# chen-zichen/distributed_learning_simulator

Measured on AMD Instinct MI355X. Metric: client-update GB/s aggregated per FL round + Shapley subset-evals/sec, higher is better.
Workload: dtype fp32; 1 GPU; FedAvg aggregation of 100 synthetic ResNet-18 (11.2M-param fp32) client updates (per GPU), bit-exact reference order; parallelism=clients sharded over 1 GPU(s) + RCCL all-reduce, clients_per_gpu=100, clients_total=100, params=11173962, padded_row=11174016

## Files before the change

### distributed_learning_simulator_amd/_native.py

```python
import ctypes
import os
import threading

import torch

_HERE = os.path.dirname(os.path.abspath(__file__))
LIB_PATH = os.environ.get("DLS_HIP_LIB", os.path.join(_HERE, "libdls_hip.so"))

FEDAVG_EXACT = 0
FEDAVG_FMA = 1
SIGN_NAN_MARK = 1 << 24
QTILE_GROUPS = 10
SUBSET_UNION_MAX = 64


def sign_words(P):
    return ((P + 255) // 256) * 8


def sign_row_pitch(P):
    return (sign_words(P) + 15) // 16 * 16


class QTile(ctypes.Structure):
# ... 31 lines not shown
    "dls_sign_sgd_direction": ([_p, _p, _i64, _f32, _f32, _i32, _i32, _p, _p, _p], _i32),
    "dls_sign_sgd_apply": ([_p, _p, _i64, _f32, _f32, _p], _i32),
    "dls_dequant_fedavg": ([_p, _i32, _p, _p, _i64, _p, _i64, _p, _i64, _i64, _p, _p, _i32, _f32,
                            _p, _p],
                           _i32),
    "dls_dequant_fedavg_mode": ([_p, _i32, _p, _p, _i64, _p, _i64, _p, _i64, _i64, _p, _p, _i32,
                                 _f32, _i32, _p, _p], _i32),
    "dls_segment_minmax_f32": ([_p, _p, _i32, _p, _p, _i64, _p], _i32),
    "dls_qparams_minmax": ([_p, _p, _i32, _i32, _i32, _i32, _p, _p, _p], _i32),
    "dls_quantize_affine": ([_p, _p, _i32, _p, _p, _i32, _i32, _p, _p, _i32, _u64, _i64, _p],
                            _i32),
    "dls_bn_fold_f32": ([_p, _p, _p, _p, _f32, _i32, _p, _p, _p], _i32),
    "dls_bn_act_nhwc_f32": ([_p, _i64, _i32, _p, _p, _p, _i32, _p, _p], _i32),
    "dls_bn_fold_exact_f32": ([_p, _p, _p, _p, _f32, _i32, _p, _p], _i32),
    "dls_bn_act_exact_nhwc_f32": ([_p, _i64, _i32, _p, _p, _i32, _p, _p], _i32),
    "dls_bn_act_exact_nchw_f32": ([_p, _i64, _i32, _i64, _p, _p, _i32, _p, _p], _i32),
    "dls_conv_pack_input_f32": ([_p, _i64, _i32, _i32, _i32, _i32, _p, _p], _i32),
    "dls_conv_pack_weights_f32": ([_p, _i32, _i32, _i32, _i32, _i32, _p, _p], _i32),
    "dls_conv_pack_im2col_f32": ([_p, _i64, _i32, _i32, _i32, _i32, _i32, _i32, _i32, _i32, _p, _p],
                                 _i32),
    "dls_conv_pack_weights_im2col_f32": ([_p, _i32, _i32, _i32, _i32, _i32, _p, _p], _i32),
    "dls_conv_bn_act_split": ([_p, _i64, _i32, _i32, _i32, _p, _i32, _i32, _i32, _i32, _i32, _p, _p,
                               _i32, _p, _p], _i32),
    "dls_conv_stem_bn_act_f32": ([_p, _i64, _i32, _i32, _i32, _p, _i32, _i32, _i32, _i32, _i32, _p,
                                  _i32, _p, _p], _i32),
    "dls_pool_linear_split": ([_p, _i64, _i32, _i32, _p, _p, _i32, _p, _p], _i32),
    "dls_conv_kernel_choice": ([_i64, _i32, _i32, _i32, _i32, _i32, _i32, _i32, _i32], _i32),
    "dls_conv_stem_kernel_choice": ([_i64, _i32, _i32, _i32, _i32, _i32, _i32, _i32, _i32], _i32),
    "dls_lenet5_eval_f32": ([_p, _i64, _i32, _p, _p, _i64, _p, _i32, _p, _p, _p], _i32),
    "dls_lenet5_eval_loss_f32": ([_p, _i64, _i32, _p, _p, _i64, _p, _i32, _p, _p, _p, _i64, _p],
                                 _i32),
    "dls_softmax_ce_f32": ([_p, _i32, _i64, _i32, _p, _p, _i64, _p], _i32),
    "dls_sum_rows_f64": ([_p, _i64, _i32, _i64, _p, _p], _i32),
}

_lib = None
_lock = threading.Lock()


def lib():
    global _lib
    if _lib is None:
        with _lock:
            if _lib is None:
                if not os.path.exists(LIB_PATH):
                    raise RuntimeError(
# ... 242 lines not shown
        return
    if (consts.dtype != torch.float32 or consts.numel() != 4 * cout or not consts.is_contiguous()
            or consts.device != device):
        raise RuntimeError(f"{fn}: consts must be a contiguous fp32 tensor of 4 * Cout = {4 * cout} "
                           f"elements on {device}")


def _overlaps(a, b):
    a0 = a.data_ptr()
    b0 = b.data_ptr()
    return a0 < b0 + b.numel() * b.element_size() and b0 < a0 + a.numel() * a.element_size()


def split_channels(c):
    return (int(c) + 31) // 32 * 32


CONV_KERNELS = {
    0: "none", 1: "generic<1,4>", 2: "generic<2,2>", 3: "pipe<1,4,10,1,2>", 4: "pipe<1,4,12,1,2>",
    5: "pipe<2,2,5,1,2>", 6: "pipe<2,4,5>", 7: "pipe<2,4,6>", 8: "halo<2,2,9,false>",
    9: "halo<2,2,9,true>", 10: "halo<1,4,11,false>", 11: "halo<1,4,11,true>", 12: "phase<2,4,5>",
}
STEM_KERNELS = {0: "none", 1: "window", 2: "3x3", 3: "generic"}


def conv_kernel_choice(B, H, W, C, Cout, ksize, stride, pad):
    kh, kw = ksize
    return int(lib().dls_conv_kernel_choice(B, H, W, C, Cout, kh, kw, stride, pad))


def conv_stem_kernel_choice(B, C, H, W, Cout, ksize, stride, pad):
    kh, kw = ksize
    return int(lib().dls_conv_stem_kernel_choice(B, C, H, W, Cout, kh, kw, stride, pad))


def conv_pack_input(x, stream=None):
    if x.dtype != torch.float32 or x.dim() != 4 or not x.is_contiguous():
        raise RuntimeError("conv_pack_input: x must be a contiguous NCHW fp32 tensor")
    B, C, H, W = x.shape
    cp = split_channels(C)
    out = torch.empty((B, H, W, 2 * cp), dtype=torch.int16, device=x.device)
    _check(lib().dls_conv_pack_input_f32(_ptr(x), B, C, H, W, cp, _ptr(out), _stream(stream, x)),
           "dls_conv_pack_input_f32")
    return out


def conv_pack_weights(w, stream=None):
    w = w.detach()
    if w.dtype != torch.float32 or w.dim() != 4 or not w.is_contiguous():
        raise RuntimeError("conv_pack_weights: w must be a contiguous fp32 [Cout, Cin, KH, KW]")
    co, ci, kh, kw = w.shape
    cp = split_channels(ci)
    out = torch.empty((co, 2 * kh * kw * cp), dtype=torch.int16, device=w.device)
    _check(lib().dls_conv_pack_weights_f32(_ptr(w), co, ci, kh, kw, cp, _ptr(out),
                                           _stream(stream, w)), "dls_conv_pack_weights_f32")
    return out
# ... 36 lines not shown
        raise RuntimeError(f"conv_bn_act: weights {tuple(w.shape)} do not match input channels {c2 // 2}")
    _check_same_device("conv_bn_act", x, w=w)
    _check_consts("conv_bn_act", consts, cout, x.device)
    oshape = (B, ho, wo, 2 * cout)
    if residual is not None:
        if (tuple(residual.shape) != oshape or residual.dtype != torch.int16
                or not residual.is_contiguous()):
            raise RuntimeError("conv_bn_act: residual must be a contiguous split NHWC int16 tensor "
                               "of the output's shape")
        _check_same_device("conv_bn_act", x, residual=residual)
    if out is None:
        out = torch.empty(oshape, dtype=torch.int16, device=x.device)
    else:
        if tuple(out.shape) != oshape or out.dtype != torch.int16 or not out.is_contiguous():
            raise RuntimeError(f"conv_bn_act: out must be a contiguous int16 tensor of shape {oshape}")
        _check_same_device("conv_bn_act", x, out=out)
        for name, t in (("x", x), ("residual", residual)):
            if t is not None and _overlaps(out, t):
                raise RuntimeError(f"conv_bn_act: out must not alias {name}")
    _check(lib().dls_conv_bn_act_split(_ptr(x), B, H, W, c2 // 2, _ptr(w), cout, kh, kw, stride,
                                       pad, _ptr(consts), _ptr(residual), int(bool(relu)),
                                       _ptr(out), _stream(stream, x)), "dls_conv_bn_act_split")
    return out


def conv_stem_bn_act(x, w, ksize, stride, pad, consts=None, relu=True, stream=None):
    if x.dtype != torch.float32 or x.dim() != 4 or not x.is_contiguous():
        raise RuntimeError("conv_stem_bn_act: x must be a contiguous NCHW fp32 tensor")
    B, C, H, W = x.shape
    kh, kw = ksize
    cout = w.shape[0]
    if w.dtype != torch.int16 or w.shape[1] != 2 * 32 or not w.is_contiguous():
        raise RuntimeError("conv_stem_bn_act: w must be conv_pack_weights_im2col output with Kp = 32")
    _check_same_device("conv_stem_bn_act", x, w=w)
    _check_consts("conv_stem_bn_act", consts, cout, x.device)
    ho, wo = (H + 2 * pad - kh) // stride + 1, (W + 2 * pad - kw) // stride + 1
    out = torch.empty((B, ho, wo, 2 * cout), dtype=torch.int16, device=x.device)
    _check(lib().dls_conv_stem_bn_act_f32(_ptr(x), B, C, H, W, _ptr(w), cout, kh, kw, stride, pad,
                                          _ptr(consts), int(bool(relu)), _ptr(out),
                                          _stream(stream, x)), "dls_conv_stem_bn_act_f32")
    return out


def pool_linear(x, weight, bias=None, stream=None):
    B, H, W, c2 = x.shape
    if x.dtype != torch.int16 or not x.is_contiguous():
# ... 131 lines not shown
```

### distributed_learning_simulator_amd/csrc/conv.hip

```cpp
#include "dls_common.h"

#include <mutex>

#ifndef DLS_CONV_GENERIC_ONLY
#define DLS_CONV_GENERIC_ONLY 0
#endif
#ifndef DLS_CONV_PHASE
#define DLS_CONV_PHASE 1
#endif
#ifndef DLS_STEM_WINDOW
#define DLS_STEM_WINDOW 1
#endif
#ifndef DLS_CONV_MF16
#define DLS_CONV_MF16 1
#endif
#ifndef DLS_STEM_TILES
#define DLS_STEM_TILES 2
#endif
#ifndef DLS_CONV_SERPENTINE
#define DLS_CONV_SERPENTINE 1
#endif
#ifndef DLS_PIPE_NARROW
#define DLS_PIPE_NARROW 1
#endif
// ... 30 lines not shown
typedef __attribute__((ext_vector_type(2))) float f32x2;

__device__ __forceinline__ void split2x2(float a, float b, uint32_t &hi2, uint32_t &lo2) {
    hi2 = __builtin_bit_cast(uint32_t, __builtin_convertvector(f32x2{a, b}, bf16x2));
    float ra = a - __uint_as_float(hi2 << 16);
    float rb = b - __uint_as_float(hi2 & 0xffff0000u);
    ra = (__float_as_uint(ra) & 0x7f800000u) == 0x7f800000u ? 0.f : ra;
    rb = (__float_as_uint(rb) & 0x7f800000u) == 0x7f800000u ? 0.f : rb;
    lo2 = __builtin_bit_cast(uint32_t, __builtin_convertvector(f32x2{ra, rb}, bf16x2));
}

struct ConvArgs {
    const uint16_t *x;
    const uint16_t *w;
    const float *consts;
    const uint16_t *res;
    uint16_t *y;
    int H, W, C, Ho, Wo, Cout, KW, taps, stride, pad, K, M, relu;
    int pix_tiles, co_tiles;
    int B, TI, TR, NH;
    int rev;
};

constexpr int kWaveTile = 64;
constexpr int kBK = 32;
constexpr int kRowB = 4 * kBK + 16;

typedef f32x16 WaveAcc[2][2];
typedef f32x4 WaveAcc16[4][4];

__device__ __forceinline__ void mfma_chunk(WaveAcc &acc, const uint8_t *arow, const uint8_t *b0,
                                           const uint8_t *b1, int h) {
    constexpr int BK = kBK, RB = kRowB;
#pragma unroll
    for (int s = 0; s < BK / 16; ++s) {
        const int off = 32 * s + 16 * h;
        bf16x8 ah[2], al[2], bh[2], bl[2];
#pragma unroll
        for (int i = 0; i < 2; ++i) {
            ah[i] = *reinterpret_cast<const bf16x8 *>(arow + i * 32 * RB + off);
            al[i] = *reinterpret_cast<const bf16x8 *>(arow + i * 32 * RB + 2 * BK + off);
        }
        bh[0] = *reinterpret_cast<const bf16x8 *>(b0 + off);
        bl[0] = *reinterpret_cast<const bf16x8 *>(b0 + 2 * BK + off);
        bh[1] = *reinterpret_cast<const bf16x8 *>(b1 + off);
        bl[1] = *reinterpret_cast<const bf16x8 *>(b1 + 2 * BK + off);
#pragma unroll
        for (int i = 0; i < 2; ++i)
#pragma unroll
            for (int j = 0; j < 2; ++j) {
                acc[i][j] = __builtin_amdgcn_mfma_f32_32x32x16_bf16(al[i], bh[j], acc[i][j], 0, 0, 0);
                acc[i][j] = __builtin_amdgcn_mfma_f32_32x32x16_bf16(ah[i], bl[j], acc[i][j], 0, 0, 0);
                acc[i][j] = __builtin_amdgcn_mfma_f32_32x32x16_bf16(ah[i], bh[j], acc[i][j], 0, 0, 0);
            }
    }
}

struct Frag {
    bf16x8 ah[2], al[2], bh[2], bl[2];
};

__device__ __forceinline__ void mfma_frag(WaveAcc &acc, const Frag &f) {
#pragma unroll
    for (int i = 0; i < 2; ++i)
#pragma unroll
        for (int j = 0; j < 2; ++j) {
            acc[i][j] = __builtin_amdgcn_mfma_f32_32x32x16_bf16(f.al[i], f.bh[j], acc[i][j], 0, 0, 0);
            acc[i][j] = __builtin_amdgcn_mfma_f32_32x32x16_bf16(f.ah[i], f.bl[j], acc[i][j], 0, 0, 0);
            acc[i][j] = __builtin_amdgcn_mfma_f32_32x32x16_bf16(f.ah[i], f.bh[j], acc[i][j], 0, 0, 0);
        }
}

__device__ __forceinline__ void zero_acc(WaveAcc &acc) {
#pragma unroll
    for (int i = 0; i < 2; ++i)
#pragma unroll
        for (int j = 0; j < 2; ++j)
#pragma unroll
            for (int e = 0; e < 16; ++e) acc[i][j][e] = 0.f;
}

template <int NPASS, int EROW>
__device__ __forceinline__ void acc_to_lds(const WaveAcc &acc, uint8_t *smem, int wc, int wp, int lane, int p) {
    const int r = lane & 31, h = lane >> 5;
#pragma unroll
    for (int j = 0; j < 2; ++j)
#pragma unroll
        for (int i = 0; i < 2; ++i) {
            if (NPASS == 2 && i != p) continue;
#pragma unroll
            for (int g = 0; g < 4; ++g) {
                const int pl = wp * kWaveTile + 32 * j + r;
// ... 677 lines not shown
            __builtin_amdgcn_sched_barrier(0);
            __builtin_amdgcn_s_waitcnt(kWaitLgkm0);
            const Frag16A cur = fa;
            if (!reload) fraga(fa, t + 1, tap == 8 ? 0 : tap + 1);
            __builtin_amdgcn_sched_barrier(0);
            mfma_half16(acc, cur, fb.bh, fb.bl, 2);
            __builtin_amdgcn_sched_barrier(0);
            retire_and_barrier<NW>(piece);
            if (reload) {
#pragma unroll
                for (int u = 0; u < NHI; ++u) issue_halo(u, cc + 1);
                retire_and_barrier<NW>(false);
                fraga(fa, t + 1, 0);
            }
        }
    }
    asm volatile("s_waitcnt vmcnt(0)" ::: "memory");
    __syncthreads();
    epilogue_lds<BMC, BNP, NT, 1, WaveAcc16>(acc, smem, a, co0, pix0, wc, wp, tid);
}

__device__ constexpr int kPhaseTap[9] = {0, 2, 6, 8, 1, 7, 3, 5, 4};

template <int WCO, int WPIX, int NHI>
__global__ __launch_bounds__(64 * WCO * WPIX, 1) void k_conv3x3s2_phase(ConvArgs a) {
    constexpr int NW = WCO * WPIX, NT = 64 * NW;
    constexpr int BMC = kWaveTile * WCO, BNP = kWaveTile * WPIX;
    constexpr int RB = 128;
    constexpr int HROWS = 8 * NW * NHI;
    constexpr int HB = HROWS * RB, AB = BMC * RB;
    constexpr int NAI = BMC / (8 * NW);
    constexpr int STAGE = 2 * HB + 3 * AB + 2 * RB;
    constexpr int EPI = BNP * (4 * BMC + 16);
    static_assert(BMC % (8 * NW) == 0 && NAI >= 1, "weight rows per wave");
    static_assert(kBK == 32, "128-byte rows");
    __shared__ __attribute__((aligned(16))) uint8_t smem[STAGE > EPI ? STAGE : EPI];
    uint8_t *const hbuf0 = smem;
    uint8_t *const abuf0 = smem + 2 * HB;
    uint8_t *const zrow = abuf0 + 3 * AB;

    const int tid = threadIdx.x, lane = tid & 63, wv = tid >> 6;
    const int wc = wv / WPIX, wp = wv % WPIX;
    int co_t, pt;
    tile_of_block(a.co_tiles, co_t, pt, a.rev);
    const int co0 = co_t * BMC;
    const int pix0 = pt * BNP;
    const int H = a.H, W = a.W, Ho = a.Ho, Wo = a.Wo, TR = a.TR;
    const int hrows_img = (TR + 1) * Wo;
    int b0, y0;
    if (TR == Ho) {
        b0 = pt * a.TI;
        y0 = 0;
    } else {
        const int tpi = Ho / TR;
        b0 = pt / tpi;
        y0 = (pt - b0 * tpi) * TR;
    }

    const int sl = lane & 7, lr = lane >> 3;
    int hpix[NHI], hpc[NHI];
#pragma unroll
    for (int u = 0; u < NHI; ++u) {
        const int hr = 8 * (u * NW + wv) + lr;
        int v = -1, s = 0;
        if (hr < a.NH) {
            const int ti = hr / hrows_img, rem = hr - ti * hrows_img;
            const int qq = rem / Wo, r = rem - qq * Wo;
            const int b = b0 + ti, q = y0 - 1 + qq;
            s = hr - ti * Wo;
            if (b < a.B && q >= 0) v = (b * H + 2 * q + 1) * W + 2 * r + 1;
        }
        hpix[u] = v;
        hpc[u] = sl ^ ((s >> 1) & 7);
    }
    const uint16_t *zero = reinterpret_cast<const uint16_t *>(kZeroPiece);
    asm volatile("" : "+s"(zero));
    const uint16_t *asrc[NAI];
#pragma unroll
    for (int u = 0; u < NAI; ++u) {
        const int row = 8 * (wv * NAI + u) + lr;
        const int p = sl ^ ((row >> 1) & 7);
        asrc[u] = a.w + (int64_t)(co0 + row) * (2 * a.K) + ((p & 4) ? a.K : 0) + 8 * (p & 3);
    }
    auto issue_weights = [&](int step, int slot) {
        const int cc = step / 9, tap = kPhaseTap[step - 9 * cc];
        const int kc = tap * a.C + cc * kBK;
        uint8_t *dst = abuf0 + (slot % 3) * AB;
#pragma unroll
        for (int u = 0; u < NAI; ++u) glds16(asrc[u] + kc, dst + (wv * NAI + u) * 8 * RB);
    };
    auto issue_halo = [&](int g) {
        const int cc = g >> 2, p = g & 3;
        const int back = (p < 2 ? 0 : W) + ((p & 1) ? 1 : 0);
#pragma unroll
        for (int u = 0; u < NHI; ++u) {
            const int v = hpix[u], pc = hpc[u];
            const uint16_t *src =
                v >= 0 ? a.x + (int64_t)(v - back) * (2 * a.C) + ((pc & 4) ? a.C : 0) + 8 * (pc & 3) + cc * kBK
                       : zero;
            glds16(src, hbuf0 + (g & 1) * HB + (u * NW + wv) * 8 * RB);
        }
    };

    const int r = lane & 31, h = lane >> 5;
    const int fa = (r >> 1) & 7;
    const int arow = (wc * kWaveTile + r) * RB;
    int hb0, pl0, ox0;
    {
        pl0 = wp * kWaveTile + r;
        const int tw = TR * Wo;
        const int ti = pl0 / tw, rem = pl0 - ti * tw;
        const int oy = rem / Wo;
        ox0 = rem - oy * Wo;
        hb0 = ti * hrows_img + oy * Wo + ox0;
    }
    const int dhb = TR * Wo >= 32 ? 32 : (32 / (TR * Wo)) * hrows_img;
    auto frag = [&](Frag &f, int step, int s) {
        const int cc = step / 9, k = step - 9 * cc;
        const int tap = kPhaseTap[k], g = 4 * cc + (k < 4 ? 0 : k < 6 ? 1 : k < 8 ? 2 : 3);
        const int ky = tap / 3, kx = tap - 3 * ky;
        const uint8_t *ab = abuf0 + (step % 3) * AB + arow;
        const uint8_t *hbb = hbuf0 + (g & 1) * HB;
        const int qh = 16 * ((2 * s + h) ^ fa), ql = 16 * ((4 + 2 * s + h) ^ fa);
#pragma unroll
        for (int i = 0; i < 2; ++i) {
            f.ah[i] = *reinterpret_cast<const bf16x8 *>(ab + i * 32 * RB + qh);
            f.al[i] = *reinterpret_cast<const bf16x8 *>(ab + i * 32 * RB + ql);
        }
        const int sh = (ky == 0 ? 0 : Wo) + (kx == 0 ? -1 : 0);
        const bool in = kx != 0 || ox0 > 0;
#pragma unroll
        for (int j = 0; j < 2; ++j) {
            const int fb = ((pl0 + 32 * j + sh) >> 1) & 7;
            const uint8_t *row = in ? hbb + (hb0 + j * dhb + sh) * RB : zrow + ((pl0 + sh) & 1) * RB;
            f.bh[j] = *reinterpret_cast<const bf16x8 *>(row + 16 * ((2 * s + h) ^ fb));
            f.bl[j] = *reinterpret_cast<const bf16x8 *>(row + 16 * ((4 + 2 * s + h) ^ fb));
        }
    };

    WaveAcc acc;
    zero_acc(acc);
    const int nc = a.C / kBK, T = 9 * nc;
    if (tid < 2 * RB / 16) *reinterpret_cast<u32x4 *>(zrow + 16 * tid) = u32x4{0u, 0u, 0u, 0u};
    issue_halo(0);
    issue_weights(0, 0);
    issue_weights(T > 1 ? 1 : 0, 1);
    retire_and_barrier<NW>(false);
    Frag f0, f1;
    frag(f0, 0, 0);
    for (int cc = 0; cc < nc; ++cc) {
#pragma unroll
        for (int k = 0; k < 9; ++k) {
            const int t = 9 * cc + k;
            const bool first = k == 0 || k == 4 || k == 6 || k == 8;
            const bool last = k == 3 || k == 5 || k == 7 || k == 8;
            const int g = 4 * cc + (k < 4 ? 0 : k < 6 ? 1 : k < 8 ? 2 : 3);
            issue_weights(t + 2 < T ? t + 2 : T - 1, t + 2);
            if (first && g + 1 < 4 * nc) issue_halo(g + 1);
            __builtin_amdgcn_s_waitcnt(kWaitLgkm0);
            frag(f1, t, 1);
            __builtin_amdgcn_sched_barrier(0);
            mfma_frag(acc, f0);
            __builtin_amdgcn_sched_barrier(0);
            if (!last) {
                __builtin_amdgcn_s_waitcnt(kWaitLgkm0);
                frag(f0, t + 1, 0);
            }
            __builtin_amdgcn_sched_barrier(0);
            mfma_frag(acc, f1);
            if (first && !last && g + 1 < 4 * nc)
                asm volatile("s_waitcnt vmcnt(%0)" ::"n"(NHI) : "memory");
            else
                asm volatile("s_waitcnt vmcnt(0)" ::: "memory");
            __builtin_amdgcn_s_barrier();
            asm volatile("" ::: "memory");
            if (last) frag(f0, t + 1, 0);
        }
    }
    asm volatile("s_waitcnt vmcnt(0)" ::: "memory");
    __syncthreads();
    epilogue_lds<BMC, BNP, NT>(acc, smem, a, co0, pix0, wc, wp, tid);
}

constexpr int kStemWinRow = 40;
template <int WPIX, int CIN = 0, int KHW = 0, bool XT = false, int NTL = 1>
__global__ __launch_bounds__(64 * WPIX) void k_conv_stem(ConvArgs a, const float *__restrict__ x) {
    constexpr int NT = 64 * WPIX, BNP = kWaveTile * WPIX;
    constexpr int STAGE = BNP * kRowB;
    constexpr int EPI = BNP * (4 * kWaveTile / 2 + 16);
    constexpr int WIN = XT ? 3 * 10 * kStemWinRow * 4 : 0;
    static_assert(NT == BNP, "one pixel row per thread");
    static_assert(!XT || (CIN == 3 && KHW == 3 && BNP == 256), "the staged window's shape");
    static_assert(NTL == 1 || XT, "tile walks: the staged-window form");
    __shared__ __attribute__((aligned(16))) uint8_t smem[(STAGE > EPI ? STAGE : EPI) + WIN];
    uint8_t *Bs = smem;
    float *win = reinterpret_cast<float *>(smem + (STAGE > EPI ? STAGE : EPI));
    const int tid = threadIdx.x, lane = tid & 63, wp = tid >> 6;
    const int r = lane & 31, h = lane >> 5;
    int co_t, pix_t;
    tile_of_block(a.co_tiles, co_t, pix_t, a.rev);
    const int co0 = co_t * kWaveTile;
    auto load_window = [&](int p0) {
        f32x4 v = f32x4{0.f, 0.f, 0.f, 0.f};
        const int b = p0 / (a.H * 32), oy0 = (p0 - b * a.H * 32) / 32;
// ... 284 lines not shown
        }
        if (DLS_CONV_PIPE && wide) {
            if (W >= 16 && fit_pipe<2, 2, 5>(a)) return DLS_CONV_KERNEL_PIPE128_W4;
            if (fit_pipe<2, 4, 5>(a)) return DLS_CONV_KERNEL_PIPE128_W8_H5;
            if (fit_pipe<2, 4, 6>(a)) return DLS_CONV_KERNEL_PIPE128_W8_H6;
        }
        if (DLS_CONV_PIPE && !wide && fit_pipe<1, 4, 10>(a)) return DLS_CONV_KERNEL_PIPE64_H10;
        const bool skew = W <= 16;
        if (wide ? fit_halo<2, 2, 9>(a) : fit_halo<1, 4, 11>(a))
            return wide ? (skew ? DLS_CONV_KERNEL_HALO128_SKEW : DLS_CONV_KERNEL_HALO128)
                        : (skew ? DLS_CONV_KERNEL_HALO64_SKEW : DLS_CONV_KERNEL_HALO64);
    }
    if (DLS_CONV_PHASE && !DLS_CONV_GENERIC_ONLY && KH == 3 && KW == 3 && a.stride == 2 && a.pad == 1 && wide &&
        fit_phase<2, 4, 5>(a))
        return DLS_CONV_KERNEL_PHASE;
    a.TI = a.TR = a.NH = 0;
    if (!(wide ? fit_generic<2, 2>(a) : fit_generic<1, 4>(a))) {
        set_error("dls_conv_bn_act_split: %lld blocks", (long long)a.pix_tiles * a.co_tiles);
        return DLS_EINVAL;
    }
    return wide ? DLS_CONV_KERNEL_GENERIC128 : DLS_CONV_KERNEL_GENERIC64;
}

inline unsigned conv_blocks(const ConvArgs &a) { return (unsigned)((int64_t)a.pix_tiles * a.co_tiles); }

template <int WCO, int WPIX>
void launch_conv(const ConvArgs &a, hipStream_t st) {
    constexpr int NBUF = WCO == 1 ? 1 : 2, NPASS = WCO == 1 ? 2 : 1;
    hipLaunchKernelGGL((k_conv_bf16x3<WCO, WPIX, NBUF, NPASS>), dim3(conv_blocks(a)), dim3(64 * WCO * WPIX), 0,
                       st, a);
}

template <int WCO, int WPIX, int NHMAX, bool SKEW>
void launch_halo(const ConvArgs &a, hipStream_t st) {
    hipLaunchKernelGGL((k_conv3x3_halo<WCO, WPIX, NHMAX, SKEW>), dim3(conv_blocks(a)), dim3(64 * WCO * WPIX), 0,
                       st, a);
}

template <int WCO, int WPIX, int NHI>
void launch_phase(const ConvArgs &a, hipStream_t st) {
    hipLaunchKernelGGL((k_conv3x3s2_phase<WCO, WPIX, NHI>), dim3(conv_blocks(a)), dim3(64 * WCO * WPIX), 0, st, a);
}

template <int WCO, int WPIX, int NHI, int NHB = 2, int OCC = 1>
void launch_pipe(const ConvArgs &a, hipStream_t st) {
    if (DLS_CONV_MF16)
        hipLaunchKernelGGL((k_conv3x3_pipe16<WCO, WPIX, NHI, NHB, OCC>), dim3(conv_blocks(a)),
                           dim3(64 * WCO * WPIX), 0, st, a);
    else
        hipLaunchKernelGGL((k_conv3x3_pipe<WCO, WPIX, NHI, NHB, OCC>), dim3(conv_blocks(a)),
                           dim3(64 * WCO * WPIX), 0, st, a);
}

int stem_choose(int C, int H, int W, int KH, int KW, int stride, int pad) {
    if (DLS_STEM_WINDOW && C == 3 && KH == 3 && KW == 3 && stride == 1 && pad == 1 && W == 32 && H % 8 == 0)
        return DLS_STEM_KERNEL_WINDOW;
    return C == 3 && KH == 3 && KW == 3 ? DLS_STEM_KERNEL_3X3 : DLS_STEM_KERNEL_GENERIC;
}

int stem_check_shape(int64_t B, int32_t C, int32_t H, int32_t W, int32_t Cout, int32_t KH, int32_t KW,
                     int32_t stride, int32_t pad, int64_t &M, int &pix_tiles, int &co_tiles) {
    DLS_REQUIRE(B >= 0 && C > 0 && H > 0 && W > 0 && KH > 0 && KW > 0 && KH * KW * C <= kBK &&
                    Cout >= 64 && Cout % 64 == 0 && stride > 0 && pad >= 0 && H + 2 * pad >= KH &&
                    W + 2 * pad >= KW,
// ... 136 lines not shown
    case DLS_CONV_KERNEL_HALO128: launch_halo<2, 2, 9, false>(a, st); break;
    case DLS_CONV_KERNEL_HALO128_SKEW: launch_halo<2, 2, 9, true>(a, st); break;
    case DLS_CONV_KERNEL_HALO64: launch_halo<1, 4, 11, false>(a, st); break;
    case DLS_CONV_KERNEL_HALO64_SKEW: launch_halo<1, 4, 11, true>(a, st); break;
    case DLS_CONV_KERNEL_PHASE: launch_phase<2, 4, 5>(a, st); break;
    case DLS_CONV_KERNEL_GENERIC128: launch_conv<2, 2>(a, st); break;
    default: launch_conv<1, 4>(a, st); break;
    }
    return check_launch("dls_conv_bn_act_split");
}

int dls_conv_kernel_choice(int64_t B, int32_t H, int32_t W, int32_t C, int32_t Cout, int32_t KH,
                           int32_t KW, int32_t stride, int32_t pad) {
    int64_t M = 0;
    if (const int rc = conv_check_shape(B, H, W, C, Cout, KH, KW, stride, pad, M)) return rc;
    if (M == 0) return DLS_CONV_KERNEL_NONE;
    const int Ho = (H + 2 * pad - KH) / stride + 1, Wo = (W + 2 * pad - KW) / stride + 1;
    ConvArgs a{nullptr, nullptr, nullptr, nullptr, nullptr, (int)H, (int)W, (int)C, Ho, Wo, (int)Cout,
               (int)KW, (int)(KH * KW), (int)stride, (int)pad, (int)(KH * KW * C), (int)M, 0, 0, 0,
               (int)B, 0, 0, 0};
    return conv_choose(a, KH);
}

int dls_conv_stem_bn_act_f32(const float *x, int64_t B, int32_t C, int32_t H, int32_t W, const uint16_t *w,
                             int32_t Cout, int32_t KH, int32_t KW, int32_t stride, int32_t pad,
                             const float *consts, int32_t relu, uint16_t *y, dls_stream_t stream) {
    DLS_REQUIRE(x && w && y, DLS_EINVAL, "dls_conv_stem_bn_act_f32: null pointer");
    int64_t M = 0;
    int pix_tiles = 0, co_tiles = 0;
    if (const int rc = stem_check_shape(B, C, H, W, Cout, KH, KW, stride, pad, M, pix_tiles, co_tiles)) return rc;
    DLS_REQUIRE(aligned16(w) && aligned16(y) && (!consts || aligned16(consts)), DLS_ELAYOUT,
                "dls_conv_stem_bn_act_f32: 16-byte alignment");
    if (M == 0) return DLS_OK;
    const int Ho = (H + 2 * pad - KH) / stride + 1, Wo = (W + 2 * pad - KW) / stride + 1;
    constexpr int WPIX = 4;
    ConvArgs a{nullptr, w, consts, nullptr, y, (int)H, (int)W, (int)C, Ho, Wo, (int)Cout, (int)KW,
               (int)(KH * KW), (int)stride, (int)pad, kBK, (int)M, relu ? 1 : 0, 0, 0, (int)B, 0, 0, 0};
    conv_record_walk(y, 0);
    a.pix_tiles = pix_tiles;
    a.co_tiles = co_tiles;
    const int64_t blocks = (int64_t)a.pix_tiles * a.co_tiles;
    switch (stem_choose(C, H, W, KH, KW, stride, pad)) {
    case DLS_STEM_KERNEL_WINDOW: {
        constexpr int NTL = DLS_STEM_TILES;
        const int64_t walks = (int64_t)((a.pix_tiles + NTL - 1) / NTL) * a.co_tiles;
        hipLaunchKernelGGL((k_conv_stem<WPIX, 3, 3, true, NTL>), dim3((unsigned)walks), dim3(64 * WPIX), 0,
// ... 36 lines not shown
```

### distributed_learning_simulator_amd/models.py

```python
import torch
import torch.nn as nn
import torch.nn.functional as F


class LeNet5(nn.Module):
    def __init__(self, num_classes=10):
        super().__init__()
        self.conv1 = nn.Conv2d(1, 6, 5)
        self.conv2 = nn.Conv2d(6, 16, 5)
        self.fc1 = nn.Linear(400, 120)
        self.fc2 = nn.Linear(120, 84)
        self.fc3 = nn.Linear(84, num_classes)

    def forward(self, x):
        x = F.max_pool2d(F.relu(self.conv1(x)), 2)
        x = F.max_pool2d(F.relu(self.conv2(x)), 2)
        x = x.flatten(1)
        return self.fc3(F.relu(self.fc2(F.relu(self.fc1(x)))))

    def split_layout(self):
        from .layout import ParameterLayout
        return ParameterLayout((n, tuple(p.shape)) for n, p in self.named_parameters())

    def split_supports(self, shape):
# ... 141 lines not shown
        for layer in (self.layer1, self.layer2, self.layer3, self.layer4):
            for blk in layer:
                s = blk.conv1.stride[0]
                ho, wo = (ho - 1) // s + 1, (wo - 1) // s + 1
                peak = max(peak, ho * wo * blk.conv1.out_channels)
        return 4 * self.conv1.in_channels * H * W + 4 * 4 * peak

    def forward_split(self, x, pk):
        from . import _native

        def cba(inp, conv, bn, residual=None, relu=True):
            return _native.conv_bn_act(inp, pk[id(conv)], conv.kernel_size, conv.stride[0],
                                       conv.padding[0], pk[id(bn)], residual, relu)

        c1 = self.conv1
        if c1.kernel_size[0] * c1.kernel_size[1] * c1.in_channels <= 32:
            out = _native.conv_stem_bn_act(x.contiguous(), pk[id(c1)], c1.kernel_size, c1.stride[0],
                                           c1.padding[0], pk[id(self.bn1)], True)
        else:
            xs = _native.conv_pack_im2col(x.contiguous(), c1.kernel_size, c1.stride[0], c1.padding[0])
            out = _native.conv_bn_act(xs, pk[id(c1)], (1, 1), 1, 0, pk[id(self.bn1)], None, True)
        for layer in (self.layer1, self.layer2, self.layer3, self.layer4):
            for blk in layer:
                h = cba(out, blk.conv1, blk.bn1)
                sc = cba(out, blk.shortcut[0], blk.shortcut[1], relu=False) if len(blk.shortcut) else out
                out = cba(h, blk.conv2, blk.bn2, residual=sc)
        lw, lb = pk[id(self.linear)]
        return _native.pool_linear(out, lw, lb)

    def forward_fused(self, x, fold):
        from . import _native
        out = _native.bn_act_exact(self.conv1(x), fold[id(self.bn1)], relu=True, inplace=True)
        for layer in (self.layer1, self.layer2, self.layer3, self.layer4):
            for blk in layer:
                out = blk.forward_fused(out, fold)
        out = F.adaptive_avg_pool2d(out, 1).flatten(1)
        return self.linear(out)


def split_conv_macs(model, H, W):
    shapes = {}
    hooks = [m.register_forward_hook(lambda m, i, o: shapes.__setitem__(id(m), o.shape))
             for m in model.modules() if isinstance(m, nn.Conv2d)]
    try:
        with torch.no_grad():
            p = next(model.parameters())
            model.eval()(torch.zeros(1, model.conv1.in_channels, H, W, device=p.device))
    finally:
# ... 25 lines not shown
```

### include/dls_hip.h

```cpp
#ifndef DLS_HIP_H
#define DLS_HIP_H

#include <stdint.h>

#ifdef __cplusplus
extern "C" {
#endif

#define DLS_ABI_VERSION 2

#define DLS_OK 0
#define DLS_EINVAL (-1)
#define DLS_ELAYOUT (-2)

#define DLS_FEDAVG_EXACT 0
#define DLS_FEDAVG_FMA 1

#define DLS_SIGN_TILE 256
#define DLS_SIGN_WORDS(P) ((((P) + 255) / 256) * 8)
#define DLS_SIGN_NAN_MARK (1 << 24)

typedef void *dls_stream_t;

const char *dls_last_error(void);
// ... 80 lines not shown
                        dls_stream_t stream);
int dls_bn_fold_exact_f32(const float *weight, const float *bias, const float *mean,
                          const float *var, float eps, int32_t C, float *consts,
                          dls_stream_t stream);
int dls_bn_act_exact_nhwc_f32(const float *x, int64_t rows, int32_t C, const float *consts,
                              const float *residual, int32_t relu, float *y, dls_stream_t stream);
int dls_bn_act_exact_nchw_f32(const float *x, int64_t N, int32_t C, int64_t HW,
                              const float *consts, const float *residual, int32_t relu, float *y,
                              dls_stream_t stream);

#define DLS_CONV_KERNEL_NONE 0
#define DLS_CONV_KERNEL_GENERIC64 1
#define DLS_CONV_KERNEL_GENERIC128 2
#define DLS_CONV_KERNEL_PIPE64_H10 3
#define DLS_CONV_KERNEL_PIPE64_H12 4
#define DLS_CONV_KERNEL_PIPE128_W4 5
#define DLS_CONV_KERNEL_PIPE128_W8_H5 6
#define DLS_CONV_KERNEL_PIPE128_W8_H6 7
#define DLS_CONV_KERNEL_HALO128 8
#define DLS_CONV_KERNEL_HALO128_SKEW 9
#define DLS_CONV_KERNEL_HALO64 10
#define DLS_CONV_KERNEL_HALO64_SKEW 11
#define DLS_CONV_KERNEL_PHASE 12
#define DLS_STEM_KERNEL_NONE 0
#define DLS_STEM_KERNEL_WINDOW 1
#define DLS_STEM_KERNEL_3X3 2
#define DLS_STEM_KERNEL_GENERIC 3
int dls_conv_kernel_choice(int64_t B, int32_t H, int32_t W, int32_t C, int32_t Cout, int32_t KH,
                           int32_t KW, int32_t stride, int32_t pad);
int dls_conv_stem_kernel_choice(int64_t B, int32_t C, int32_t H, int32_t W, int32_t Cout, int32_t KH,
                                int32_t KW, int32_t stride, int32_t pad);
int dls_conv_pack_input_f32(const float *x, int64_t B, int32_t C, int32_t H, int32_t W, int32_t Cp,
                            uint16_t *out, dls_stream_t stream);
int dls_conv_pack_weights_f32(const float *w, int32_t Cout, int32_t Cin, int32_t KH, int32_t KW,
                              int32_t Cp, uint16_t *out, dls_stream_t stream);
int dls_conv_pack_im2col_f32(const float *x, int64_t B, int32_t C, int32_t H, int32_t W, int32_t KH,
                             int32_t KW, int32_t stride, int32_t pad, int32_t Kp, uint16_t *out,
                             dls_stream_t stream);
int dls_conv_pack_weights_im2col_f32(const float *w, int32_t Cout, int32_t Cin, int32_t KH, int32_t KW,
                                     int32_t Kp, uint16_t *out, dls_stream_t stream);
int dls_conv_bn_act_split(const uint16_t *x, int64_t B, int32_t H, int32_t W, int32_t C,
                          const uint16_t *w, int32_t Cout, int32_t KH, int32_t KW, int32_t stride,
                          int32_t pad, const float *consts, const uint16_t *residual, int32_t relu,
                          uint16_t *y, dls_stream_t stream);
int dls_conv_stem_bn_act_f32(const float *x, int64_t B, int32_t C, int32_t H, int32_t W, const uint16_t *w,
                             int32_t Cout, int32_t KH, int32_t KW, int32_t stride, int32_t pad,
                             const float *consts, int32_t relu, uint16_t *y, dls_stream_t stream);
int dls_pool_linear_split(const uint16_t *x, int64_t B, int32_t HW, int32_t C, const float *weight,
                          const float *bias, int32_t O, float *out, dls_stream_t stream);

int dls_lenet5_eval_f32(const float *models, int64_t ldm, int32_t S, const int64_t *offsets,
                        const float *x, int64_t B, const int64_t *labels, int32_t O,
                        float *logits, int64_t *correct, dls_stream_t stream);

int dls_softmax_ce_f32(const float *logits, int32_t S, int64_t B, int32_t O, const int64_t *labels,
                       float *loss, int64_t ldn, dls_stream_t stream);
int dls_lenet5_eval_loss_f32(const float *models, int64_t ldm, int32_t S, const int64_t *offsets,
                             const float *x, int64_t B, const int64_t *labels, int32_t O,
                             float *logits, int64_t *correct, float *loss, int64_t ldn,
                             dls_stream_t stream);
int dls_sum_rows_f64(const float *v, int64_t ldn, int32_t S, int64_t n, double *out,
                     dls_stream_t stream);

#ifdef __cplusplus
}
#endif
#endif
// ... 1 lines not shown
```

Before: 6724 GB/s.

## Fuse the 1x1 strided shortcut conv into the 3x3 stride-2 phase conv kernel

Adds a paired kernel variant of the stride-2 phase conv. It loads the 1x1 shortcut weights once per channel chunk and reuses the centre-tap halo fragments to accumulate the shortcut output in a second accumulator, then writes both through the LDS epilogue. The ResNet forward uses it for downsampling blocks, so the shortcut conv no longer needs its own launch and its own read of the input activations. In exchange it costs more LDS per stage, a second accumulator's worth of registers, and an extra epilogue pass. It only affects the ResNet forward used for Shapley evaluation, not the FedAvg aggregation.

Measured after the change: 6722 GB/s (median of 3 runs). Within noise of the previous version (-0.0%).

```diff
diff --git a/distributed_learning_simulator_amd/_native.py b/distributed_learning_simulator_amd/_native.py
--- a/distributed_learning_simulator_amd/_native.py
+++ b/distributed_learning_simulator_amd/_native.py
@@ -77,6 +77,9 @@
     "dls_conv_pack_weights_im2col_f32": ([_p, _i32, _i32, _i32, _i32, _i32, _p, _p], _i32),
     "dls_conv_bn_act_split": ([_p, _i64, _i32, _i32, _i32, _p, _i32, _i32, _i32, _i32, _i32, _p, _p,
                                _i32, _p, _p], _i32),
+    "dls_conv_bn_act_pair_split": ([_p, _i64, _i32, _i32, _i32, _p, _i32, _i32, _i32, _i32, _i32, _p, _p,
+                                    _i32, _p, _p, _p, _p, _p], _i32),
+    "dls_conv_pair_kernel_choice": ([_i64, _i32, _i32, _i32, _i32, _i32, _i32, _i32, _i32], _i32),
     "dls_conv_stem_bn_act_f32": ([_p, _i64, _i32, _i32, _i32, _p, _i32, _i32, _i32, _i32, _i32, _p,
                                   _i32, _p, _p], _i32),
     "dls_pool_linear_split": ([_p, _i64, _i32, _i32, _p, _p, _i32, _p, _p], _i32),
@@ -365,6 +368,8 @@
     9: "halo<2,2,9,true>", 10: "halo<1,4,11,false>", 11: "halo<1,4,11,true>", 12: "phase<2,4,5>",
 }
 STEM_KERNELS = {0: "none", 1: "window", 2: "3x3", 3: "generic"}
+CONV_PAIR_PHASE_SC = 13
+CONV_PAIR_KERNELS = {CONV_PAIR_PHASE_SC: "phase<2,4,5,true>"}
 
 
 def conv_kernel_choice(B, H, W, C, Cout, ksize, stride, pad):
@@ -375,6 +380,11 @@
 def conv_stem_kernel_choice(B, C, H, W, Cout, ksize, stride, pad):
     kh, kw = ksize
     return int(lib().dls_conv_stem_kernel_choice(B, C, H, W, Cout, kh, kw, stride, pad))
+
+
+def conv_pair_kernel_choice(B, H, W, C, Cout, ksize, stride, pad):
+    kh, kw = ksize
+    return int(lib().dls_conv_pair_kernel_choice(B, H, W, C, Cout, kh, kw, stride, pad))
 
 
 def conv_pack_input(x, stream=None):
@@ -457,6 +467,28 @@
                                        pad, _ptr(consts), _ptr(residual), int(bool(relu)),
                                        _ptr(out), _stream(stream, x)), "dls_conv_bn_act_split")
     return out
+
+
+def conv_bn_act_pair(x, w, ksize, stride, pad, consts, w_sc, consts_sc, relu=True, stream=None):
+    B, H, W, c2 = x.shape
+    kh, kw = ksize
+    cout = w.shape[0]
+    ho, wo = (H + 2 * pad - kh) // stride + 1, (W + 2 * pad - kw) // stride + 1
+    if any(t.dtype != torch.int16 or not t.is_contiguous() for t in (x, w, w_sc)):
+        raise RuntimeError("conv_bn_act_pair: split int16 contiguous operands expected")
+    if w.shape[1] != kh * kw * c2 or tuple(w_sc.shape) != (cout, c2):
+        raise RuntimeError(f"conv_bn_act_pair: weights {tuple(w.shape)} / shortcut weights "
+                           f"{tuple(w_sc.shape)} do not match {c2 // 2} input and {cout} output channels")
+    _check_same_device("conv_bn_act_pair", x, w=w, w_sc=w_sc)
+    _check_consts("conv_bn_act_pair", consts, cout, x.device)
+    _check_consts("conv_bn_act_pair", consts_sc, cout, x.device)
+    y = torch.empty((B, ho, wo, 2 * cout), dtype=torch.int16, device=x.device)
+    y_sc = torch.empty_like(y)
+    _check(lib().dls_conv_bn_act_pair_split(_ptr(x), B, H, W, c2 // 2, _ptr(w), cout, kh, kw, stride,
+                                            pad, _ptr(consts), None, int(bool(relu)), _ptr(y),
+                                            _ptr(w_sc), _ptr(consts_sc), _ptr(y_sc),
+                                            _stream(stream, x)), "dls_conv_bn_act_pair_split")
+    return y, y_sc
 
 
 def conv_stem_bn_act(x, w, ksize, stride, pad, consts=None, relu=True, stream=None):
diff --git a/distributed_learning_simulator_amd/csrc/conv.hip b/distributed_learning_simulator_amd/csrc/conv.hip
--- a/distributed_learning_simulator_amd/csrc/conv.hip
+++ b/distributed_learning_simulator_amd/csrc/conv.hip
@@ -76,6 +76,15 @@
     int rev;
 };
 
+struct ShortcutArgs {
+    const uint16_t *w;
+    const float *consts;
+    uint16_t *y;
+};
+struct NoShortcut {};
+__device__ __forceinline__ NoShortcut shortcut_of() { return {}; }
+__device__ __forceinline__ const ShortcutArgs &shortcut_of(const ShortcutArgs &s) { return s; }
+
 constexpr int kWaveTile = 64;
 constexpr int kBK = 32;
 constexpr int kRowB = 4 * kBK + 16;
@@ -122,6 +131,17 @@
             acc[i][j] = __builtin_amdgcn_mfma_f32_32x32x16_bf16(f.al[i], f.bh[j], acc[i][j], 0, 0, 0);
             acc[i][j] = __builtin_amdgcn_mfma_f32_32x32x16_bf16(f.ah[i], f.bl[j], acc[i][j], 0, 0, 0);
             acc[i][j] = __builtin_amdgcn_mfma_f32_32x32x16_bf16(f.ah[i], f.bh[j], acc[i][j], 0, 0, 0);
+        }
+}
+
+__device__ __forceinline__ void mfma_frag_ab(WaveAcc &acc, const Frag &fa, const Frag &fb) {
+#pragma unroll
+    for (int i = 0; i < 2; ++i)
+#pragma unroll
+        for (int j = 0; j < 2; ++j) {
+            acc[i][j] = __builtin_amdgcn_mfma_f32_32x32x16_bf16(fa.al[i], fb.bh[j], acc[i][j], 0, 0, 0);
+            acc[i][j] = __builtin_amdgcn_mfma_f32_32x32x16_bf16(fa.ah[i], fb.bl[j], acc[i][j], 0, 0, 0);
+            acc[i][j] = __builtin_amdgcn_mfma_f32_32x32x16_bf16(fa.ah[i], fb.bh[j], acc[i][j], 0, 0, 0);
         }
 }
 
@@ -845,15 +865,17 @@
 
 __device__ constexpr int kPhaseTap[9] = {0, 2, 6, 8, 1, 7, 3, 5, 4};
 
-template <int WCO, int WPIX, int NHI>
-__global__ __launch_bounds__(64 * WCO * WPIX, 1) void k_conv3x3s2_phase(ConvArgs a) {
+template <int WCO, int WPIX, int NHI, bool FUSE_SC = false, class... SC>
+__global__ __launch_bounds__(64 * WCO * WPIX, 1) void k_conv3x3s2_phase(ConvArgs a, SC... sc_arg) {
+    static_assert(sizeof...(SC) == (FUSE_SC ? 1 : 0), "the shortcut's operands with FUSE_SC only");
+    const auto &sc = shortcut_of(sc_arg...);
     constexpr int NW = WCO * WPIX, NT = 64 * NW;
     constexpr int BMC = kWaveTile * WCO, BNP = kWaveTile * WPIX;
     constexpr int RB = 128;
     constexpr int HROWS = 8 * NW * NHI;
     constexpr int HB = HROWS * RB, AB = BMC * RB;
     constexpr int NAI = BMC / (8 * NW);
-    constexpr int STAGE = 2 * HB + 3 * AB + 2 * RB;
+    constexpr int STAGE = 2 * HB + (FUSE_SC ? 4 : 3) * AB + 2 * RB;
     constexpr int EPI = BNP * (4 * BMC + 16);
     static_assert(BMC % (8 * NW) == 0 && NAI >= 1, "weight rows per wave");
     static_assert(kBK == 32, "128-byte rows");
@@ -861,6 +883,7 @@
     uint8_t *const hbuf0 = smem;
     uint8_t *const abuf0 = smem + 2 * HB;
     uint8_t *const zrow = abuf0 + 3 * AB;
+    uint8_t *const scbuf = zrow + 2 * RB;
 
     const int tid = threadIdx.x, lane = tid & 63, wv = tid >> 6;
     const int wc = wv / WPIX, wp = wv % WPIX;
@@ -895,33 +918,76 @@
         }
         hpix[u] = v;
         hpc[u] = sl ^ ((s >> 1) & 7);
+        if constexpr (FUSE_SC) hpix[u] = v >= 0 ? v * 8 + hpc[u] : -1;
     }
     const uint16_t *zero = reinterpret_cast<const uint16_t *>(kZeroPiece);
     asm volatile("" : "+s"(zero));
     const uint16_t *asrc[NAI];
+    int aoff[NAI];
 #pragma unroll
     for (int u = 0; u < NAI; ++u) {
         const int row = 8 * (wv * NAI + u) + lr;
         const int p = sl ^ ((row >> 1) & 7);
         asrc[u] = a.w + (int64_t)(co0 + row) * (2 * a.K) + ((p & 4) ? a.K : 0) + 8 * (p & 3);
+        aoff[u] = (co0 + row) * (2 * a.K) + ((p & 4) ? a.K : 0) + 8 * (p & 3);
     }
     auto issue_weights = [&](int step, int slot) {
         const int cc = step / 9, tap = kPhaseTap[step - 9 * cc];
-        const int kc = tap * a.C + cc * kBK;
+        int Cv = a.C;
+        if constexpr (FUSE_SC) asm volatile("" : "+s"(Cv));
+        const int kc = tap * Cv + cc * kBK;
         uint8_t *dst = abuf0 + (slot % 3) * AB;
 #pragma unroll
-        for (int u = 0; u < NAI; ++u) glds16(asrc[u] + kc, dst + (wv * NAI + u) * 8 * RB);
+        for (int u = 0; u < NAI; ++u) {
+            if constexpr (FUSE_SC)
+                glds16(a.w + (aoff[u] + kc), dst + (wv * NAI + u) * 8 * RB);
+            else
+                glds16(asrc[u] + kc, dst + (wv * NAI + u) * 8 * RB);
+        }
     };
     auto issue_halo = [&](int g) {
         const int cc = g >> 2, p = g & 3;
-        const int back = (p < 2 ? 0 : W) + ((p & 1) ? 1 : 0);
+        int Wv = W;
+        if constexpr (FUSE_SC) asm volatile("" : "+s"(Wv));
+        auto C = [&] {
+            if constexpr (FUSE_SC) {
+                int c = a.C;
+                asm volatile("" : "+s"(c));
+                return c;
+            } else {
+                return a.C;
+            }
+        };
+        const int back = (p < 2 ? 0 : Wv) + ((p & 1) ? 1 : 0);
 #pragma unroll
         for (int u = 0; u < NHI; ++u) {
-            const int v = hpix[u], pc = hpc[u];
+            int v, pc;
+            if constexpr (FUSE_SC) {
+                int hv = hpix[u];
+                asm volatile("" : "+v"(hv));
+                v = hv >> 3;
+                pc = hv & 7;
+            } else {
+                v = hpix[u];
+                pc = hpc[u];
+            }
             const uint16_t *src =
-                v >= 0 ? a.x + (int64_t)(v - back) * (2 * a.C) + ((pc & 4) ? a.C : 0) + 8 * (pc & 3) + cc * kBK
+                v >= 0 ? a.x + (int64_t)(v - back) * (2 * C()) + ((pc & 4) ? C() : 0) + 8 * (pc & 3) + cc * kBK
                        : zero;
             glds16(src, hbuf0 + (g & 1) * HB + (u * NW + wv) * 8 * RB);
+        }
+    };
+    auto issue_shortcut = [&](int cc) {
+        if constexpr (FUSE_SC) {
+#pragma unroll
+            for (int u = 0; u < NAI; ++u) {
+                const int row = 8 * (wv * NAI + u) + lr;
+                const int p = sl ^ ((row >> 1) & 7);
+                int Cv = a.C;
+                asm volatile("" : "+s"(Cv));
+                glds16(sc.w + ((co0 + row) * (2 * Cv) + ((p & 4) ? Cv : 0) + 8 * (p & 3) + cc * kBK),
+                       scbuf + (wv * NAI + u) * 8 * RB);
+            }
         }
     };
 
@@ -950,19 +1016,31 @@
             f.ah[i] = *reinterpret_cast<const bf16x8 *>(ab + i * 32 * RB + qh);
             f.al[i] = *reinterpret_cast<const bf16x8 *>(ab + i * 32 * RB + ql);
         }
-        const int sh = (ky == 0 ? 0 : Wo) + (kx == 0 ? -1 : 0);
+        int Wov = Wo, dhbv = dhb;
+        if constexpr (FUSE_SC) asm volatile("" : "+s"(Wov), "+s"(dhbv));
+        const int sh = (ky == 0 ? 0 : Wov) + (kx == 0 ? -1 : 0);
         const bool in = kx != 0 || ox0 > 0;
 #pragma unroll
         for (int j = 0; j < 2; ++j) {
             const int fb = ((pl0 + 32 * j + sh) >> 1) & 7;
-            const uint8_t *row = in ? hbb + (hb0 + j * dhb + sh) * RB : zrow + ((pl0 + sh) & 1) * RB;
+            const uint8_t *row = in ? hbb + (hb0 + j * dhbv + sh) * RB : zrow + ((pl0 + sh) & 1) * RB;
             f.bh[j] = *reinterpret_cast<const bf16x8 *>(row + 16 * ((2 * s + h) ^ fb));
             f.bl[j] = *reinterpret_cast<const bf16x8 *>(row + 16 * ((4 + 2 * s + h) ^ fb));
         }
     };
+    auto frag_shortcut = [&](Frag &f, int s) {
+        const int qh = 16 * ((2 * s + h) ^ fa), ql = 16 * ((4 + 2 * s + h) ^ fa);
+#pragma unroll
+        for (int i = 0; i < 2; ++i) {
+            f.ah[i] = *reinterpret_cast<const bf16x8 *>(scbuf + arow + i * 32 * RB + qh);
+            f.al[i] = *reinterpret_cast<const bf16x8 *>(scbuf + arow + i * 32 * RB + ql);
+        }
+    };
 
     WaveAcc acc;
     zero_acc(acc);
+    WaveAcc acc_sc;
+    if constexpr (FUSE_SC) zero_acc(acc_sc);
     const int nc = a.C / kBK, T = 9 * nc;
     if (tid < 2 * RB / 16) *reinterpret_cast<u32x4 *>(zrow + 16 * tid) = u32x4{0u, 0u, 0u, 0u};
     issue_halo(0);
@@ -980,18 +1058,42 @@
             const int g = 4 * cc + (k < 4 ? 0 : k < 6 ? 1 : k < 8 ? 2 : 3);
             issue_weights(t + 2 < T ? t + 2 : T - 1, t + 2);
             if (first && g + 1 < 4 * nc) issue_halo(g + 1);
+            const bool scw = FUSE_SC && k == 0, scm = FUSE_SC && k == 8;
+            if (scw) issue_shortcut(cc);
             __builtin_amdgcn_s_waitcnt(kWaitLgkm0);
-            frag(f1, t, 1);
-            __builtin_amdgcn_sched_barrier(0);
-            mfma_frag(acc, f0);
-            __builtin_amdgcn_sched_barrier(0);
-            if (!last) {
+            if (scm) {
+                Frag fs;
+                frag_shortcut(fs, 0);
+                __builtin_amdgcn_sched_barrier(0);
+                mfma_frag(acc, f0);
+                __builtin_amdgcn_sched_barrier(0);
                 __builtin_amdgcn_s_waitcnt(kWaitLgkm0);
-                frag(f0, t + 1, 0);
+                frag(f1, t, 1);
+                __builtin_amdgcn_sched_barrier(0);
+                mfma_frag_ab(acc_sc, fs, f0);
+                __builtin_amdgcn_sched_barrier(0);
+                __builtin_amdgcn_s_waitcnt(kWaitLgkm0);
+                frag_shortcut(fs, 1);
+                __builtin_amdgcn_sched_barrier(0);
+                mfma_frag(acc, f1);
+                __builtin_amdgcn_sched_barrier(0);
+                __builtin_amdgcn_s_waitcnt(kWaitLgkm0);
+                mfma_frag_ab(acc_sc, fs, f1);
+            } else {
+                frag(f1, t, 1);
+                __builtin_amdgcn_sched_barrier(0);
+                mfma_frag(acc, f0);
+                __builtin_amdgcn_sched_barrier(0);
+                if (!last) {
+                    __builtin_amdgcn_s_waitcnt(kWaitLgkm0);
+                    frag(f0, t + 1, 0);
+                }
+                __builtin_amdgcn_sched_barrier(0);
+                mfma_frag(acc, f1);
             }
-            __builtin_amdgcn_sched_barrier(0);
-            mfma_frag(acc, f1);
-            if (first && !last && g + 1 < 4 * nc)
+            if (scw)
+                asm volatile("s_waitcnt vmcnt(%0)" ::"n"(NHI + NAI) : "memory");
+            else if (first && !last && g + 1 < 4 * nc)
                 asm volatile("s_waitcnt vmcnt(%0)" ::"n"(NHI) : "memory");
             else
                 asm volatile("s_waitcnt vmcnt(0)" ::: "memory");
@@ -1003,6 +1105,15 @@
     asm volatile("s_waitcnt vmcnt(0)" ::: "memory");
     __syncthreads();
     epilogue_lds<BMC, BNP, NT>(acc, smem, a, co0, pix0, wc, wp, tid);
+    if constexpr (FUSE_SC) {
+        ConvArgs s = a;
+        s.consts = sc.consts;
+        s.res = nullptr;
+        s.relu = 0;
+        s.y = sc.y;
+        __syncthreads();
+        epilogue_lds<BMC, BNP, NT>(acc_sc, smem, s, co0, pix0, wc, wp, tid);
+    }
 }
 
 constexpr int kStemWinRow = 40;
@@ -1333,6 +1444,33 @@
     return wide ? DLS_CONV_KERNEL_GENERIC128 : DLS_CONV_KERNEL_GENERIC64;
 }
 
+int conv_pair_check_shape(int64_t B, int32_t H, int32_t W, int32_t C, int32_t Cout, int32_t KH, int32_t KW,
+                          int32_t stride, int32_t pad, int64_t &M) {
+    int64_t Msc = 0;
+    if (const int rc = conv_check_shape(B, H, W, C, Cout, KH, KW, stride, pad, M)) return rc;
+    if (const int rc = conv_check_shape(B, H, W, C, Cout, 1, 1, stride, 0, Msc)) return rc;
+    DLS_REQUIRE((H + 2 * pad - KH) / stride == (H - 1) / stride && (W + 2 * pad - KW) / stride == (W - 1) / stride,
+                DLS_EINVAL,
+                "dls_conv_bn_act_pair_split: KH=%d KW=%d stride=%d pad=%d over %dx%d: the 1x1 shortcut's "
+                "output has another shape",
+                KH, KW, stride, pad, H, W);
+    return DLS_OK;
+}
+
+int conv_pair_choose(ConvArgs &a, int KH) {
+    const int id = conv_choose(a, KH);
+    if (id < 0) return id;
+    if (id == DLS_CONV_KERNEL_PHASE && (int64_t)a.B * a.H * a.W < (1ll << 28) &&
+        (int64_t)a.Cout * 2 * a.K < (1ll << 31))
+        return DLS_CONV_PAIR_KERNEL_PHASE_SC;
+    ConvArgs s = a;
+    s.KW = s.taps = 1;
+    s.pad = 0;
+    s.K = a.C;
+    const int id_sc = conv_choose(s, 1);
+    return id_sc < 0 ? id_sc : id;
+}
+
 inline unsigned conv_blocks(const ConvArgs &a) { return (unsigned)((int64_t)a.pix_tiles * a.co_tiles); }
 
 template <int WCO, int WPIX>
@@ -1351,6 +1489,12 @@
 template <int WCO, int WPIX, int NHI>
 void launch_phase(const ConvArgs &a, hipStream_t st) {
     hipLaunchKernelGGL((k_conv3x3s2_phase<WCO, WPIX, NHI>), dim3(conv_blocks(a)), dim3(64 * WCO * WPIX), 0, st, a);
+}
+
+template <int WCO, int WPIX, int NHI>
+void launch_phase_shortcut(const ConvArgs &a, const ShortcutArgs &sc, hipStream_t st) {
+    hipLaunchKernelGGL((k_conv3x3s2_phase<WCO, WPIX, NHI, true, ShortcutArgs>), dim3(conv_blocks(a)), dim3(64 * WCO * WPIX), 0,
+                       st, a, sc);
 }
 
 template <int WCO, int WPIX, int NHI, int NHB = 2, int OCC = 1>
@@ -1533,6 +1677,51 @@
     return conv_choose(a, KH);
 }
 
+int dls_conv_bn_act_pair_split(const uint16_t *x, int64_t B, int32_t H, int32_t W, int32_t C,
+                               const uint16_t *w, int32_t Cout, int32_t KH, int32_t KW, int32_t stride,
+                               int32_t pad, const float *consts, const uint16_t *residual, int32_t relu,
+                               uint16_t *y, const uint16_t *w_sc, const float *consts_sc, uint16_t *y_sc,
+                               dls_stream_t stream) {
+    DLS_REQUIRE(x && w && y && w_sc && y_sc, DLS_EINVAL, "dls_conv_bn_act_pair_split: null pointer");
+    int64_t M = 0;
+    if (const int rc = conv_pair_check_shape(B, H, W, C, Cout, KH, KW, stride, pad, M)) return rc;
+    DLS_REQUIRE(aligned16(x) && aligned16(w) && aligned16(y) && (!consts || aligned16(consts)) &&
+                    (!residual || aligned16(residual)) && aligned16(w_sc) && aligned16(y_sc) &&
+                    (!consts_sc || aligned16(consts_sc)),
+                DLS_ELAYOUT, "dls_conv_bn_act_pair_split: 16-byte alignment");
+    if (M == 0) return DLS_OK;
+    const int Ho = (H + 2 * pad - KH) / stride + 1, Wo = (W + 2 * pad - KW) / stride + 1;
+    ConvArgs a{x, w, consts, residual, y, (int)H, (int)W, (int)C, Ho, Wo, (int)Cout, (int)KW,
+               (int)(KH * KW), (int)stride, (int)pad, (int)(KH * KW * C), (int)M, relu ? 1 : 0, 0, 0,
+               (int)B, 0, 0, 0};
+    const int id = conv_pair_choose(a, KH);
+    if (id < 0) return id;
+    if (id != DLS_CONV_PAIR_KERNEL_PHASE_SC) {
+        if (const int rc = dls_conv_bn_act_split(x, B, H, W, C, w, Cout, KH, KW, stride, pad, consts, residual,
+                                                 relu, y, stream))
+            return rc;
+        return dls_conv_bn_act_split(x, B, H, W, C, w_sc, Cout, 1, 1, stride, 0, consts_sc, nullptr, 0, y_sc,
+                                     stream);
+    }
+    a.rev = conv_walk_direction(x);
+    conv_record_walk(y, a.rev);
+    conv_record_walk(y_sc, a.rev);
+    launch_phase_shortcut<2, 4, 5>(a, ShortcutArgs{w_sc, consts_sc, y_sc}, as_stream(stream));
+    return check_launch("dls_conv_bn_act_pair_split");
+}
+
+int dls_conv_pair_kernel_choice(int64_t B, int32_t H, int32_t W, int32_t C, int32_t Cout, int32_t KH,
+                                int32_t KW, int32_t stride, int32_t pad) {
+    int64_t M = 0;
+    if (const int rc = conv_pair_check_shape(B, H, W, C, Cout, KH, KW, stride, pad, M)) return rc;
+    if (M == 0) return DLS_CONV_KERNEL_NONE;
+    const int Ho = (H + 2 * pad - KH) / stride + 1, Wo = (W + 2 * pad - KW) / stride + 1;
+    ConvArgs a{nullptr, nullptr, nullptr, nullptr, nullptr, (int)H, (int)W, (int)C, Ho, Wo, (int)Cout,
+               (int)KW, (int)(KH * KW), (int)stride, (int)pad, (int)(KH * KW * C), (int)M, 0, 0, 0,
+               (int)B, 0, 0, 0};
+    return conv_pair_choose(a, KH);
+}
+
 int dls_conv_stem_bn_act_f32(const float *x, int64_t B, int32_t C, int32_t H, int32_t W, const uint16_t *w,
                              int32_t Cout, int32_t KH, int32_t KW, int32_t stride, int32_t pad,
                              const float *consts, int32_t relu, uint16_t *y, dls_stream_t stream) {
diff --git a/distributed_learning_simulator_amd/models.py b/distributed_learning_simulator_amd/models.py
--- a/distributed_learning_simulator_amd/models.py
+++ b/distributed_learning_simulator_amd/models.py
@@ -187,8 +187,14 @@
             out = _native.conv_bn_act(xs, pk[id(c1)], (1, 1), 1, 0, pk[id(self.bn1)], None, True)
         for layer in (self.layer1, self.layer2, self.layer3, self.layer4):
             for blk in layer:
-                h = cba(out, blk.conv1, blk.bn1)
-                sc = cba(out, blk.shortcut[0], blk.shortcut[1], relu=False) if len(blk.shortcut) else out
+                if len(blk.shortcut):
+                    c, s = blk.conv1, blk.shortcut[0]
+                    if s.kernel_size != (1, 1) or s.padding != (0, 0) or s.stride != c.stride:
+                        raise RuntimeError("forward_split: a 1x1 unpadded shortcut of conv1's stride expected")
+                    h, sc = _native.conv_bn_act_pair(out, pk[id(c)], c.kernel_size, c.stride[0], c.padding[0],
+                                                     pk[id(blk.bn1)], pk[id(s)], pk[id(blk.shortcut[1])])
+                else:
+                    h, sc = cba(out, blk.conv1, blk.bn1), out
                 out = cba(h, blk.conv2, blk.bn2, residual=sc)
         lw, lb = pk[id(self.linear)]
         return _native.pool_linear(out, lw, lb)
diff --git a/include/dls_hip.h b/include/dls_hip.h
--- a/include/dls_hip.h
+++ b/include/dls_hip.h
@@ -126,6 +126,7 @@
 #define DLS_CONV_KERNEL_HALO64 10
 #define DLS_CONV_KERNEL_HALO64_SKEW 11
 #define DLS_CONV_KERNEL_PHASE 12
+#define DLS_CONV_PAIR_KERNEL_PHASE_SC 13
 #define DLS_STEM_KERNEL_NONE 0
 #define DLS_STEM_KERNEL_WINDOW 1
 #define DLS_STEM_KERNEL_3X3 2
@@ -147,6 +148,13 @@
                           const uint16_t *w, int32_t Cout, int32_t KH, int32_t KW, int32_t stride,
                           int32_t pad, const float *consts, const uint16_t *residual, int32_t relu,
                           uint16_t *y, dls_stream_t stream);
+int dls_conv_bn_act_pair_split(const uint16_t *x, int64_t B, int32_t H, int32_t W, int32_t C,
+                               const uint16_t *w, int32_t Cout, int32_t KH, int32_t KW, int32_t stride,
+                               int32_t pad, const float *consts, const uint16_t *residual, int32_t relu,
+                               uint16_t *y, const uint16_t *w_sc, const float *consts_sc, uint16_t *y_sc,
+                               dls_stream_t stream);
+int dls_conv_pair_kernel_choice(int64_t B, int32_t H, int32_t W, int32_t C, int32_t Cout, int32_t KH,
+                                int32_t KW, int32_t stride, int32_t pad);
 int dls_conv_stem_bn_act_f32(const float *x, int64_t B, int32_t C, int32_t H, int32_t W, const uint16_t *w,
                              int32_t Cout, int32_t KH, int32_t KW, int32_t stride, int32_t pad,
                              const float *consts, int32_t relu, uint16_t *y, dls_stream_t stream);
```
